# zeehu/generative_ranking_recommender

Measured on NVIDIA B200. Metric: RQ-KMeans vectors/sec per iteration (512-d, [128,128,256]), higher is better.
Workload: dtype 3xTF32 distance (fp32 accumulate), fp16 auction, fp32 centroids

## Files before the change

generative_ranking_recommender_b200/csrc/auction.cu:

```cuda
#include "common.cuh"

namespace rqk {

constexpr int AUC_W = 256;
constexpr int AUC_HALF = AUC_W / 2;
constexpr int AUC_NBUF = 3;
constexpr int AUC_BPL = AUC_W / 32;
constexpr int AUC_NW = 16;
constexpr int AUC_THREADS = AUC_NW * 32;
constexpr int AUC_BASE_CTAS = 296;
constexpr int AUC_MAX_CTAS = 1024;
constexpr int AUC_MAX_JOBS_PER_CTA = 65024;
constexpr int AUC_MIN_TILES_PER_CTA = 2;
constexpr int AUC_COLD_SHIFT = 8;
constexpr int AUC_MIN_KEY = 0x0400;
constexpr int AUC_SUB = 4096;
constexpr int AUC_QCAP = 256;
constexpr int AUC_SAMPLE_MAX = 8192;
constexpr int AUC_SEG_CAP = 256;
constexpr int AUC_KH = 128;
constexpr int AUC_SAMPLE_THREADS = 512;

enum { MODE_HIST = 0, MODE_BID = 1, MODE_DONE = 2 };

__device__ __forceinline__ void pdl_launch_dependents() { asm volatile("griddepcontrol.launch_dependents;" ::: "memory"); }
__device__ __forceinline__ void pdl_wait() { asm volatile("griddepcontrol.wait;" ::: "memory"); }

struct AuctionState {
    int mode;
    int counter;
    int rounds;
    int done;
    int ff_pending;
    int frozen_exit;
    int passes;
    int cold_passes;
    int window_misses;
    unsigned int eps_bits;
    unsigned int smax_bits, smin_bits;
    int need_sample;
    int error;
    int use_list;
    int force_scan;
    int list_passes;
    int sink[4];
    int branch[4];
    int pad_[4];
};

struct AuctionPtrs {
    AuctionState* st;
    __half* cost;
    short* owner;
    __half* sown;
    unsigned int* hist_g;
    unsigned int* above_g;
    unsigned int* gap_g;
    unsigned int* n_with;
    unsigned int* n_viol;
    unsigned int* tie_total;
    int* win_base;
    int* win_hbase;
    int* win_nlo;
    int* win_shift;
    int* tkey;
    int* take;
    int* tprev;
    int* miss_run;
    unsigned int* tieprefix;
    unsigned short* hist_cta;
    unsigned int* seg_list;
    unsigned int* seg_cnt;
    int* list_ok;
    unsigned int* rank_off;
    unsigned int* ticket;
    int* res_pass;
    unsigned int* above_cta;
    unsigned int* gap_cta;
    int* unres_g;
};

static inline int auction_tile_cols(int K) { return K <= 128 ? 128 : 64; }

static inline int auction_grid(long long N, int K) {
    long long tiles = ceil_div<long long>(N, auction_tile_cols(K));
    long long g = ceil_div<long long>(tiles, AUC_MIN_TILES_PER_CTA);
    const char* e = getenv("RQK_AUCTION_GRID");
    const int cap = (e && atoi(e) >= 1 && atoi(e) <= AUC_BASE_CTAS) ? atoi(e) : AUC_BASE_CTAS;
    if (g > cap) g = cap;
    long long g16 = ceil_div<long long>(N, AUC_MAX_JOBS_PER_CTA);
    if (g < g16) g = g16;
    if (g < 1) g = 1;
    return (int)g;
}

static inline int auction_spc(long long N, int K) {
    const int J = auction_tile_cols(K), G = auction_grid(N, K);
    const long long tiles = ceil_div<long long>(N, J);
    const long long len = ceil_div<long long>(tiles, G) * J;
    return (int)ceil_div<long long>(len, AUC_SUB);
}

static inline size_t auction_ws_layout(long long N, long long ld, int K, AuctionPtrs* p, char* base,
                                       size_t* reduce_off = nullptr, size_t* tie_total_off = nullptr) {
    int G = auction_grid(N, K);
    size_t off = 0;
    auto take_ = [&](size_t bytes) { size_t o = off; off += align256(bytes); return o; };
    size_t o_st = take_(sizeof(AuctionState));
    size_t o_cost = take_((size_t)ld * 2);
    size_t o_own = take_((size_t)ld * 2);
    size_t o_sown = take_((size_t)ld * 2);
    size_t o_hist = take_(((size_t)K * AUC_W + 2 * K + 2) * 4);
    size_t o_tt = take_((size_t)K * 4);
    size_t o_wb = take_((size_t)K * 4);
    size_t o_whb = take_((size_t)K * 4);
    size_t o_wnl = take_((size_t)K * 4);
    size_t o_ws = take_((size_t)K * 4);
    size_t o_tk = take_((size_t)K * 4);
    size_t o_take = take_((size_t)K * 4);
    size_t o_tprev = take_((size_t)K * 4);
    size_t o_mr = take_((size_t)K * 4);
    size_t o_tp = take_((size_t)G * K * 4);
    size_t o_hc = take_((size_t)G * K * AUC_W * 2);
    const size_t nseg = (size_t)G * auction_spc(N, K);
    size_t o_sl = take_(nseg * K * AUC_SEG_CAP * 4);
    size_t o_sc = take_(nseg * K * 4);
    size_t o_lo = take_(4);
    size_t o_ro = take_((size_t)K * 4);
    size_t o_tk2 = take_(4);
    size_t o_rp = take_((size_t)K * 4);
    size_t o_ac = take_((size_t)G * K * 4);
    size_t o_gc = take_((size_t)G * K * 4);
    size_t o_ug = take_(16);
    if (reduce_off) *reduce_off = o_hist;
    if (tie_total_off) *tie_total_off = o_tt;
    if (p) {
        p->st = (AuctionState*)(base + o_st);
        p->cost = (__half*)(base + o_cost);
        p->owner = (short*)(base + o_own);
        p->sown = (__half*)(base + o_sown);
        p->hist_g = (unsigned int*)(base + o_hist);
        p->above_g = p->hist_g + (size_t)K * AUC_W;
        p->gap_g = p->above_g + K;
        p->n_with = p->gap_g + K;
        p->n_viol = p->n_with + 1;
        p->tie_total = (unsigned int*)(base + o_tt);
        p->win_base = (int*)(base + o_wb);
        p->win_hbase = (int*)(base + o_whb);
        p->win_nlo = (int*)(base + o_wnl);
        p->win_shift = (int*)(base + o_ws);
        p->tkey = (int*)(base + o_tk);
        p->take = (int*)(base + o_take);
        p->tprev = (int*)(base + o_tprev);
        p->miss_run = (int*)(base + o_mr);
        p->tieprefix = (unsigned int*)(base + o_tp);
        p->hist_cta = (unsigned short*)(base + o_hc);
        p->seg_list = (unsigned int*)(base + o_sl);
        p->seg_cnt = (unsigned int*)(base + o_sc);
        p->list_ok = (int*)(base + o_lo);
        p->rank_off = (unsigned int*)(base + o_ro);
        p->ticket = (unsigned int*)(base + o_tk2);
        p->res_pass = (int*)(base + o_rp);
        p->above_cta = (unsigned int*)(base + o_ac);
        p->gap_cta = (unsigned int*)(base + o_gc);
        p->unres_g = (int*)(base + o_ug);
    }
    return off;
}

__global__ void auction_init_kernel(AuctionPtrs p, long long ld, int K, const unsigned int* minmax_keys, int force_scan) {
    long long i = (long long)blockIdx.x * blockDim.x + threadIdx.x;
    long long stride = (long long)gridDim.x * blockDim.x;
    for (long long j = i; j < ld; j += stride) {
        p.cost[j] = __ushort_as_half(0);
        p.owner[j] = -1;
    }
    for (long long j = i; j < (long long)K * AUC_W + 2 * K + 2; j += stride) p.hist_g[j] = 0;
    for (long long j = i; j < K; j += stride) {
        p.win_base[j] = 0;
        p.win_hbase[j] = AUC_HALF;
        p.win_nlo[j] = AUC_HALF;
        p.win_shift[j] = AUC_COLD_SHIFT;
        p.tkey[j] = -1;
        p.take[j] = 0;
        p.tprev[j] = -1;
        p.miss_run[j] = 0;
        p.rank_off[j] = 0;
        p.res_pass[j] = -1;
    }
    if (i == 0) {
        AuctionState s;
        memset(&s, 0, sizeof(s));
        s.mode = MODE_HIST;
        s.need_sample = 1;
        s.force_scan = force_scan;
        *p.list_ok = 1;
        *p.ticket = 0;
        p.unres_g[0] = 0;
        p.unres_g[1] = 0;
        p.unres_g[2] = 0;
// ... 851 lines not shown
                uint4 bufA[4], bufB[4];
                int a = warp, st = 0;
                int w = a < nact ? (int)acth[a] : 0;
                if (a < nact) load_step(w, 0, bufA);
                auto body = [&](uint4 (&cur)[4], uint4 (&nxt)[4]) {
                    int an = a, wn = w, sn = st + 1;
                    if (sn == nsteps) { an = a + AUC_NW; sn = 0; wn = an < nact ? (int)acth[an] : 0; }
                    if (an < nact) load_step(wn, sn, nxt);
                    const __half2 f2 = u2h2(sm.r_lo2[w]);
                    const uint4* cp = reinterpret_cast<const uint4*>(cost_s) + (st << 7) + lane;
                    unsigned int acc = 0;
#pragma unroll
                    for (int q = 0; q < 4; ++q) {
                        const uint4 cv = cp[q * 32];
                        const unsigned int sw[4] = {cur[q].x, cur[q].y, cur[q].z, cur[q].w};
                        const unsigned int cw[4] = {cv.x, cv.y, cv.z, cv.w};
#pragma unroll
                        for (int h = 0; h < 4; ++h) {
                            const __half2 v2 = __hsub2(u2h2(sw[h]), u2h2(cw[h]));
                            acc |= __hge2_mask(v2, f2) & ((1u << (4 * q + h)) | (1u << (16 + 4 * q + h)));
                        }
                    }
                    const int mine = __popc(acc);
                    int incl = mine;
#pragma unroll
                    for (int d = 1; d < 32; d <<= 1) {
                        const int o = __shfl_up_sync(0xffffffffu, incl, d);
                        if (lane >= d) incl += o;
                    }
                    const int total = __shfl_sync(0xffffffffu, incl, 31);
                    if (total) {
                        const int cbase = (st << 10) + lane * 8;
                        if (qn + total > AUC_QCAP) flush(w);
                        if (total <= AUC_QCAP) {
                            int pos = qn + incl - mine;
                            while (acc) {
                                const int bpos = __ffs(acc) - 1;
                                acc &= acc - 1;
                                const int pq = bpos & 15;
                                wq[pos++] = (unsigned short)(cbase + ((pq >> 2) << 8) + ((pq & 3) << 1) + (bpos >> 4));
                            }
                            qn += total;
                        } else {
                            while (__any_sync(0xffffffffu, acc != 0)) {
                                const int pc = __popc(acc);
                                const int take = pc < 4 ? pc : 4;
                                int in2 = take;
#pragma unroll
                                for (int d = 1; d < 32; d <<= 1) {
                                    const int o = __shfl_up_sync(0xffffffffu, in2, d);
                                    if (lane >= d) in2 += o;
                                }
                                int pos = in2 - take;
                                for (int r = 0; r < take; ++r) {
                                    const int bpos = __ffs(acc) - 1;
                                    acc &= acc - 1;
                                    const int pq = bpos & 15;
                                    wq[pos++] = (unsigned short)(cbase + ((pq >> 2) << 8) + ((pq & 3) << 1) + (bpos >> 4));
                                }
                                qn = __shfl_sync(0xffffffffu, in2, 31);
                                flush(w);
                            }
                        }
                    }
                    if (sn == 0 && qn) flush(w);
                    a = an;
                    w = wn;
                    st = sn;
                };
                while (a < nact) {
                    body(bufA, bufB);
#pragma unroll
                    for (int q = 0; q < 4; ++q) bufA[q] = bufB[q];
                }
            } else {
                for (int a = warp; a < nact; a += AUC_NW) {
                    const int w = acth[a];
                    const __half* srow = S + (size_t)w * ld + sub;
                    const int wbase = sm.r_base[w];
                    if (wbase > 0) {
                        const int whb = sm.r_hbase[w], wnlo = sm.r_nlo[w], wshift = sm.r_shift[w];
                        const __half lo = bits2h(key2h((unsigned)wbase));
                        for (int c0 = 0; c0 < sublen; c0 += 32) {
                            const int cc = c0 + lane;
                            bool live = cc < sublen;
                            if (live) live = __hge(__hsub(srow[cc], __ushort_as_half(cost_s[cc])), lo);
                            if (__any_sync(0xffffffffu, live)) emit(w, srow, live, live ? cc : 0, wbase, whb, wnlo, wshift);
                        }
                    } else {
                        const int shift = sm.r_shift[w];
                        for (int c0 = 0; c0 < sublen; c0 += 32) {
                            const int cc = c0 + lane;
                            const bool valid = cc < sublen;
                            __half v = __ushort_as_half(0xfc00);
                            if (valid) {
                                const __half sx = srow[cc];
                                v = (own_s[cc] == w) ? sx : __hsub(sx, __ushort_as_half(cost_s[cc]));
                            }
                            const int bin = (int)h2key(h2bits(v)) >> shift;
                            const bool hb = valid && bin < AUC_W;
                            const bool ab = valid && bin >= AUC_W;
                            unsigned int na = __popc(__ballot_sync(0xffffffffu, ab));
                            if (lane == 0 && na) atomicAdd(&sm.above[w], na);
                            unsigned int actm = __ballot_sync(0xffffffffu, hb);
                            if (actm) {
                                int lead = __ffs(actm) - 1;
                                int lbin = __shfl_sync(0xffffffffu, bin, lead);
                                unsigned int same = __ballot_sync(0xffffffffu, hb && bin == lbin);
                                if (same == actm) {
                                    if (lane == lead) hist_add(sm.hist, w - h0, lbin, __popc(actm));
                                } else if (hb) {
                                    hist_add(sm.hist, w - h0, bin);
                                }
                            }
                        }
                    }
                }
            }
            __syncthreads();
            if (tid >= h0 && tid < h0 + AUC_KH && tid < K && sm.r_shift[tid] != 0xff) {
                const unsigned int c = seg_cnt_s[tid];
                p.seg_cnt[(size_t)seg * K + tid] = c;
                if (c > AUC_SEG_CAP) *p.list_ok = 0;
            }
        }

        unsigned int* dump = reinterpret_cast<unsigned int*>(p.hist_cta + ((size_t)b * K + h0) * AUC_W);
        for (int a = tid >> 7; a < nact; a += AUC_THREADS >> 7) {
            const int i = ((int)acth[a] - h0) * (AUC_W / 2) + (tid & 127);
            const unsigned int h = sm.hist[i];
            dump[i] = h;
            if (!fused) {
                const int ig = h0 * (AUC_W / 2) + i;
                if (h & 0xffffu) atomicAdd(&p.hist_g[2 * ig], h & 0xffffu);
                if (h >> 16) atomicAdd(&p.hist_g[2 * ig + 1], h >> 16);
            }
        }
        ffh = 0;
    }

    const int nact_all = s_act_off[2];
    for (int a = tid; a < nact_all; a += AUC_THREADS) {
        const int i = act[a];
        if (fused) {
            p.above_cta[(size_t)b * K + i] = sm.above[i];
            p.gap_cta[(size_t)b * K + i] = sm.gap[i];
        } else {
            if (sm.above[i]) atomicAdd(&p.above_g[i], sm.above[i]);
            if (sm.gap[i]) atomicAdd(&p.gap_g[i], sm.gap[i]);
        }
    }
}

__global__ void __launch_bounds__(AUC_THREADS, 2)
auction_bidlist_kernel(const __half* __restrict__ S, long long ld, long long N, int K, int J, int spc, AuctionPtrs p,
                       long long n_global, int fused) {
    pdl_launch_dependents();
    pdl_wait();
    const AuctionState st = *p.st;
    if (st.mode != MODE_BID || !st.use_list) return;
    constexpr int NCH = AUC_SEG_CAP / 32;
    __shared__ __align__(16) unsigned int colmax[AUC_SUB];
    __shared__ __align__(16) short own_s[AUC_SUB];
    __shared__ __align__(16) unsigned char colviol[AUC_SUB];
    __shared__ unsigned int tie_seen[256];
    __shared__ int r_take[256], r_tk[256];
    __shared__ unsigned int s_nwith, s_nviol;
    const int tid = threadIdx.x, lane = tid & 31, warp = tid >> 5;
    const int counter = st.counter;
    const __half eps = bits2h(st.eps_bits);
    const unsigned int eps_bits = st.eps_bits;
    const bool retain = counter >= 1 && counter < 100;
    const bool fallback = counter > 1000;
    const int G = gridDim.x, b = blockIdx.x;
    const long long tiles_total = (N + J - 1) / J;
    const long long c_begin = (tiles_total * b / G) * J;
    long long c_end = (tiles_total * (b + 1) / G) * J;
    if (c_end > N) c_end = N;

    for (int i = tid; i < K; i += AUC_THREADS) {
        tie_seen[i] = p.tieprefix[(size_t)b * K + i];
        r_tk[i] = p.tkey[i];
        r_take[i] = p.take[i];
    }
    if (tid == 0) { s_nwith = 0; s_nviol = 0; }

    int seg = b * spc;
    for (long long sub = c_begin; sub < c_end; sub += AUC_SUB, ++seg) {
        const int sublen = (int)((c_end - sub) < AUC_SUB ? (c_end - sub) : AUC_SUB);
        static_assert(AUC_SUB == 8 * AUC_THREADS, "one 8-job group per thread");
        const int j0 = tid * 8;
        const bool grp = j0 < sublen;
        uint4 c8 = make_uint4(0u, 0u, 0u, 0u), o8 = make_uint4(0xffffffffu, 0xffffffffu, 0xffffffffu, 0xffffffffu);
        if (grp) {
            c8 = *reinterpret_cast<const uint4*>(p.cost + sub + j0);
            o8 = *reinterpret_cast<const uint4*>(p.owner + sub + j0);
        }
        {
            const unsigned int ow[4] = {o8.x, o8.y, o8.z, o8.w};
            unsigned int init[8];
#pragma unroll
            for (int e = 0; e < 8; ++e) {
                const int o = (int)(short)((ow[e >> 1] >> ((e & 1) * 16)) & 0xffffu);
                unsigned int v = 0;
                if (j0 + e < sublen) {
                    if (o >= 0) { if (retain) v = (eps_bits << 16) | (0xffffu - (unsigned)o); }
                    else if (fallback) v = (eps_bits << 16) | 0xffffu;
                }
                init[e] = v;
            }
            *reinterpret_cast<uint4*>(own_s + j0) = o8;
            *reinterpret_cast<uint4*>(colmax + j0) = make_uint4(init[0], init[1], init[2], init[3]);
            *reinterpret_cast<uint4*>(colmax + j0 + 4) = make_uint4(init[4], init[5], init[6], init[7]);
            *reinterpret_cast<uint2*>(colviol + j0) = make_uint2(0u, 0u);
        }
        __syncthreads();
        const int nrows = (K - warp + AUC_NW - 1) / AUC_NW;
        unsigned int E_l = (lane < nrows) ? __ldcg(p.seg_cnt + (size_t)seg * K + warp + AUC_NW * lane) : 0u;
        if (E_l > AUC_SEG_CAP) E_l = AUC_SEG_CAP;
        unsigned int pre0 = 0, pre1 = 0;
        {
            const unsigned int E0 = __shfl_sync(0xffffffffu, E_l, 0);
            const unsigned int* L0 = p.seg_list + ((size_t)seg * K + warp) * AUC_SEG_CAP;
            if ((unsigned)lane < E0) pre0 = __ldcg(L0 + lane);
            if ((unsigned)lane + 32 < E0) pre1 = __ldcg(L0 + 32 + lane);
        }
        for (int r = 0; r < nrows; ++r) {
            const int w = warp + AUC_NW * r;
            const unsigned int E = __shfl_sync(0xffffffffu, E_l, r);
            const unsigned int* L = p.seg_list + ((size_t)seg * K + w) * AUC_SEG_CAP;
            const int tk = r_tk[w];
            const __half T = bits2h(key2h((unsigned)tk));
            unsigned int ent[NCH], tmask[NCH];
            unsigned int n_ties = 0;
            ent[0] = pre0;
            ent[1] = pre1;
#pragma unroll
            for (int c = 2; c < NCH; ++c) {
                ent[c] = 0u;
                if ((unsigned)(c * 32) < E) {
                    const unsigned int idx = c * 32 + lane;
                    if (idx < E) ent[c] = __ldcg(L + idx);
                }
            }
            pre0 = 0; pre1 = 0;
            if (r + 1 < nrows) {
                const unsigned int En = __shfl_sync(0xffffffffu, E_l, r + 1);
                const unsigned int* Ln = L + (size_t)AUC_NW * AUC_SEG_CAP;
                if ((unsigned)lane < En) pre0 = __ldcg(Ln + lane);
                if ((unsigned)lane + 32 < En) pre1 = __ldcg(Ln + 32 + lane);
            }
#pragma unroll
            for (int c = 0; c < NCH; ++c) {
                tmask[c] = 0u;
                if ((unsigned)(c * 32) < E) {
                    const unsigned int idx = c * 32 + lane;
                    tmask[c] = __ballot_sync(0xffffffffu, idx < E && (int)(ent[c] & 0xffffu) == tk);
                    n_ties += __popc(tmask[c]);
                }
            }
            const unsigned int seen0 = tie_seen[w];
            const long long quota = r_take[w];
            const bool all_rej = (long long)seen0 >= quota;
            const bool all_acc = (long long)seen0 + n_ties <= quota;
            unsigned int rank[NCH];
#pragma unroll
            for (int c = 0; c < NCH; ++c) rank[c] = 0;
            if (n_ties && !all_rej && !all_acc) {
#pragma unroll
                for (int c = 0; c < NCH; ++c) {
                    unsigned int m = tmask[c];
                    while (m) {
                        const int src = __ffs(m) - 1;
                        m &= m - 1;
                        const unsigned int jsrc = __shfl_sync(0xffffffffu, ent[c], src) >> 16;
#pragma unroll
                        for (int c2 = 0; c2 < NCH; ++c2) rank[c2] += ((ent[c2] >> 16) > jsrc) ? 1u : 0u;
                    }
                }
            }
#pragma unroll
            for (int c = 0; c < NCH; ++c) {
                if ((unsigned)(c * 32) >= E) break;
                const unsigned int idx = c * 32 + lane;
                if (idx >= E) continue;
                const int key = (int)(ent[c] & 0xffffu);
                const int cc = (int)(ent[c] >> 16);
                bool bidder = key > tk;
                if (key == tk) bidder = all_acc || (!all_rej && (long long)seen0 + rank[c] < quota);
                if (!bidder) continue;
                const int o = own_s[cc];
                const bool own = (o == w);
                if (fallback && w == 0 && o < 0) continue;
                const __half v = bits2h(key2h((unsigned)key));
                unsigned int bid = h2bits(__hadd(__hsub(v, T), eps));
                if (retain && own) bid = eps_bits;
                if (!own) colviol[cc] = 1;
                atomicMax(&colmax[cc], (bid << 16) | (0xffffu - (unsigned)w));
            }
            if (lane == 0) tie_seen[w] = seen0 + n_ties;
        }
        __syncthreads();
        {
            const uint4 pa = *reinterpret_cast<const uint4*>(colmax + j0), pb = *reinterpret_cast<const uint4*>(colmax + j0 + 4);
            const uint2 vi = *reinterpret_cast<const uint2*>(colviol + j0);
            const unsigned int pk[8] = {pa.x, pa.y, pa.z, pa.w, pb.x, pb.y, pb.z, pb.w};
            const unsigned int cw[4] = {c8.x, c8.y, c8.z, c8.w}, ow[4] = {o8.x, o8.y, o8.z, o8.w};
            unsigned short sv[8];
            unsigned int changed = 0;
#pragma unroll
            for (int e = 0; e < 8; ++e) {
                sv[e] = 0;
                const int old_owner = (int)(short)((ow[e >> 1] >> ((e & 1) * 16)) & 0xffffu);
                if (pk[e]) {
                    const int wnr = (int)(0xffffu - (pk[e] & 0xffffu));
                    if (wnr != old_owner) {
                        changed |= 1u << e;
                        sv[e] = __half_as_ushort(S[(size_t)wnr * ld + sub + j0 + e]);
                    }
                }
            }
            unsigned int nc[4], no[4];
            int n_has = 0, n_vv = 0;
            bool cost_dirty = false, own_dirty = false;
#pragma unroll
            for (int e = 0; e < 8; ++e) {
                const int sh = (e & 1) * 16;
                unsigned int c = (cw[e >> 1] >> sh) & 0xffffu, o = (ow[e >> 1] >> sh) & 0xffffu;
                const int old_owner = (int)(short)o;
                bool vv = ((e < 4 ? vi.x >> (8 * e) : vi.y >> (8 * (e - 4))) & 0xffu) != 0;
                if (pk[e]) {
                    ++n_has;
                    c = h2bits(__hadd(__ushort_as_half((unsigned short)c), bits2h(pk[e] >> 16)));
                    cost_dirty = true;
                    if ((changed >> e) & 1u) { o = 0xffffu - (pk[e] & 0xffffu); own_dirty = true; }
                } else if (old_owner >= 0) {
                    o = 0xffffu;
                    own_dirty = true;
                    vv = true;
                }
                n_vv += vv ? 1 : 0;
                if (e & 1) { nc[e >> 1] |= c << 16; no[e >> 1] |= o << 16; }
                else { nc[e >> 1] = c; no[e >> 1] = o; }
            }
            if (grp) {
                if (cost_dirty) *reinterpret_cast<uint4*>(p.cost + sub + j0) = make_uint4(nc[0], nc[1], nc[2], nc[3]);
                if (own_dirty) *reinterpret_cast<uint4*>(p.owner + sub + j0) = make_uint4(no[0], no[1], no[2], no[3]);
#pragma unroll
                for (int e = 0; e < 8; ++e)
                    if ((changed >> e) & 1u) p.sown[sub + j0 + e] = __ushort_as_half(sv[e]);
            }
            n_has = __reduce_add_sync(0xffffffffu, n_has);
            n_vv = __reduce_add_sync(0xffffffffu, n_vv);
            if (lane == 0) {
                if (n_has) atomicAdd(&s_nwith, (unsigned)n_has);
                if (n_vv) atomicAdd(&s_nviol, (unsigned)n_vv);
            }
        }
        __syncthreads();
    }
    if (tid == 0) {
        if (s_nwith) atomicAdd(p.n_with, s_nwith);
        if (s_nviol) atomicAdd(p.n_viol, s_nviol);
    }
    if (fused && auction_last_cta(p.ticket)) auction_resolve_body(p, n_global, K, n_global / K, MODE_BID);
}

static inline size_t auction_pass_smem(int K, int J) {
    return (size_t)AUC_NBUF * K * J * 2 + (size_t)K * 16 + (size_t)J * 4 +
           (size_t)J * 4 + (size_t)K * 2 + (size_t)J + 64;
}

constexpr int AUC_SAMPLE = AUC_SAMPLE_MAX;
__device__ __forceinline__ void sample_select_bin(const unsigned int* hist, int base, int need, int* out_bin, int* out_above) {
    const int lane = threadIdx.x & 31;
    int h[8], lsum = 0;
#pragma unroll
    for (int i = 0; i < 8; ++i) { h[i] = (int)hist[lane * 8 + i]; lsum += h[i]; }
    int suf = lsum;
#pragma unroll
    for (int d = 1; d < 32; d <<= 1) {
        const int o = __shfl_down_sync(0xffffffffu, suf, d);
        if (lane + d < 32) suf += o;
    }
    int c = base + suf - lsum, bin = -1, above = 0;
#pragma unroll
    for (int i = 7; i >= 0; --i) {
        if (bin < 0 && c + h[i] >= need) { bin = lane * 8 + i; above = c; }
        c += h[i];
    }
    const unsigned int who = __ballot_sync(0xffffffffu, bin >= 0);
    int rb = 0, ra = base + __shfl_sync(0xffffffffu, suf, 0);
    if (who) {
        const int src = 31 - __clz(who);
        rb = __shfl_sync(0xffffffffu, bin, src);
        ra = __shfl_sync(0xffffffffu, above, src);
    }
    if (lane == 0) { *out_bin = rb; *out_above = ra; }
    *out_bin = rb;
    *out_above = ra;
}



__global__ void __launch_bounds__(AUC_SAMPLE_THREADS, 2)
auction_sample_kernel(const __half* __restrict__ S, long long ld, long long N, int K, long long jpw, AuctionPtrs p,
                      unsigned short* __restrict__ collect_out, int collect_n,
                      const unsigned short* __restrict__ ext_keys, int ext_n, int ext_cnt, PeerCtx peers, int peer_seq) {
    pdl_launch_dependents();
    pdl_wait();
    const AuctionState st = *p.st;
    if (st.mode != MODE_HIST || !st.need_sample) return;
    __shared__ unsigned short keys[AUC_SAMPLE];
    const int w = blockIdx.x, tid = threadIdx.x;
    if (peers.world > 0) {
        if (!peer_barrier(peers, 0, peer_seq, blockIdx.x == 0)) {
            if (tid == 0) { p.st->error = 1; p.st->mode = MODE_DONE; p.st->done = 1; }
            return;
        }
    }
    long long ns = N < AUC_SAMPLE ? N : AUC_SAMPLE;
    if (collect_out) ns = collect_n < ns ? collect_n : ns;
    if (ext_keys || peers.world > 0) ns = ext_n;
    const __half eps = bits2h(st.eps_bits);
    {
        constexpr int PER = 8;
        static_assert(AUC_SAMPLE % (PER * AUC_SAMPLE_THREADS) == 0, "whole batches");
        const long long nchunks = (ns + 15) / 16, cstride = N / (nchunks > 0 ? nchunks : 1);
        for (int q0 = 0; q0 < AUC_SAMPLE / AUC_SAMPLE_THREADS; q0 += PER) {
            __half c_r[PER], s_r[PER];
            short o_r[PER];
            unsigned short k_r[PER];
#pragma unroll
            for (int q = 0; q < PER; ++q) {
                const int i = tid + (q0 + q) * AUC_SAMPLE_THREADS;
                k_r[q] = 0;
                c_r[q] = s_r[q] = __ushort_as_half(0);
                o_r[q] = -1;
                if (ext_keys || peers.world > 0) {
                    if (i < ns) {
                        if (peers.world > 0)
                            k_r[q] = __ldcv(peer_sample(peers, i / ext_cnt, K, peer_seq & 1) + (size_t)w * ext_cnt + (i % ext_cnt));
                        else
                            k_r[q] = ext_keys[((size_t)(i / ext_cnt) * K + w) * ext_cnt + (i % ext_cnt)];
                    }
                } else if (i < ns) {
                    long long col = cstride * (i >> 4) + (i & 15);
                    if (col >= N) col = N - 1;
                    c_r[q] = p.cost[col];
                    o_r[q] = p.owner[col];
                    s_r[q] = S[(size_t)w * ld + col];
                }
            }
#pragma unroll
// ... 476 lines not shown
    if (s_mode != MODE_HIST) return;
    if (p.tkey[w] < 0) {
        unsigned int abt, gpt;
        merge_worker_dumps(p, K, G, w, m, &abt, &gpt);
        unsigned int* mine = peer_hist(peers, peers.rank, K, seq & 1);
        if (tid < AUC_W) mine[(size_t)w * AUC_W + tid] = m.hist[tid];
        if (tid == 0) { mine[(size_t)K * AUC_W + w] = abt; mine[(size_t)K * AUC_W + K + w] = gpt; }
    }
    __threadfence_system();
    __syncthreads();
    if (tid == 0) {
        const int t = atomicAdd(&p.unres_g[2], 1);
        s_mode = (t == (int)gridDim.x - 1) ? 1 : 0;
        if (s_mode) p.unres_g[2] = 0;
    }
    __syncthreads();
    if (s_mode && tid < peers.world && tid != peers.rank) {
        __threadfence_system();
        int* dst = peer_flags(peers, tid) + 1 * PEER_MAX + peers.rank;
        asm volatile("st.release.sys.global.s32 [%0], %1;" ::"l"(dst), "r"(seq) : "memory");
    }
}

__global__ void __launch_bounds__(AUC_MAX_CTAS, 1)
auction_peer_resolve_workers_kernel(AuctionPtrs p, int K, int G, long long jpw, PeerCtx peers, int seq) {
    pdl_launch_dependents();
    pdl_wait();
    __shared__ MergeSmem m;
    __shared__ unsigned int s_rows[PEER_MAX][AUC_W];
    __shared__ unsigned int s_abgp[2][PEER_MAX];
    __shared__ int s_flag[2], s_mode, s_passes;
    const int w = blockIdx.x, tid = threadIdx.x, warp = tid >> 5, par = seq & 1;
    if (tid == 0) { s_mode = p.st->mode; s_passes = p.st->passes; s_flag[0] = 0; s_flag[1] = 0; }
    __syncthreads();
    if (s_mode != MODE_HIST) return;
    const bool settled = p.tkey[w] >= 0;
    if (!settled) {
        if (!peer_barrier(peers, 1, seq, false)) {
            if (tid == 0) { p.st->error = 1; p.st->mode = MODE_DONE; p.st->done = 1; }
            return;
        }
        for (int i = tid; i < PEER_MAX * AUC_W; i += AUC_MAX_CTAS) {
            const int r = i / AUC_W, b = i % AUC_W;
            unsigned int v = 0;
            if (r < peers.world) {
                const unsigned int* src = peer_hist(peers, r, K, par) + (size_t)w * AUC_W + b;
                v = (r == peers.rank) ? __ldcg(src) : __ldcv(src);
            }
            s_rows[r][b] = v;
        }
        if (tid < 2 * PEER_MAX) {
            const int r = tid % PEER_MAX, which = tid / PEER_MAX;
            unsigned int v = 0;
            if (r < peers.world) {
                const unsigned int* src = peer_hist(peers, r, K, par) + (size_t)K * AUC_W + (size_t)which * K + w;
                v = (r == peers.rank) ? __ldcg(src) : __ldcv(src);
            }
            s_abgp[which][r] = v;
        }
        __syncthreads();
        if (tid < AUC_W) {
            unsigned int t = 0;
#pragma unroll
            for (int r = 0; r < PEER_MAX; ++r) t += s_rows[r][tid];
            m.hist[tid] = t;
        }
        __syncthreads();
        if (warp == 0) {
            unsigned long long abt = 0, gpt = 0;
#pragma unroll
            for (int r = 0; r < PEER_MAX; ++r) { abt += s_abgp[0][r]; gpt += s_abgp[1][r]; }
            resolve_worker_from_smem(p, w, m, abt, gpt, jpw, s_passes, s_flag);
        }
        __syncthreads();
        const int tk = p.tkey[w];
        if (tk >= 0) {
            const int base = p.win_base[w], hbase = p.win_hbase[w], nlo = p.win_nlo[w];
            const int bin = tk >= hbase ? nlo + tk - hbase : tk - base;
            unsigned int off = 0;
            for (int r = 0; r < peers.rank; ++r) off += s_rows[r][bin];
            if (tid == 0) p.rank_off[w] = off;
            tie_prefix_worker(p, K, G, w, m, off);
        }
        if (tid == 0) {
            if (s_flag[0]) atomicAdd(&p.unres_g[0], 1);
            if (s_flag[1]) atomicAdd(&p.unres_g[1], 1);
        }
    }
    if (auction_last_cta(p.ticket) && tid == 0) merge_state_transition(p);
}

__global__ void auction_tie_offset_kernel(AuctionPtrs p, int K, int G, const int* __restrict__ totals, int rank) {
    if (p.st->mode != MODE_BID) return;
    int i = blockIdx.x * blockDim.x + threadIdx.x;
    if (i < G * K) {
        unsigned int off = 0;
        for (int r = 0; r < rank; ++r) off += (unsigned int)totals[r * K + i % K];
        p.tieprefix[i] += off;
    }
}

__global__ void auction_finalize_kernel(AuctionPtrs p, long long N, int* __restrict__ assign) {
    long long i = (long long)blockIdx.x * blockDim.x + threadIdx.x;
    if (i < N) {
        short o = p.owner[i];
        assign[i] = o >= 0 ? (int)o : 0;
    }
}

}

namespace rqk {
struct AuctionArgs {
    AuctionPtrs p;
    int G, J;
    size_t smem;
};
static int auction_prepare(int64_t n, int64_t ld, int32_t k, void* workspace, size_t workspace_bytes, AuctionArgs* a,
                           const char* who) {
    if (!workspace) return fail(RQK_ERR_ARG, "%s: null workspace", who);
    if (k < 1 || k > 256) return fail(RQK_ERR_UNSUPPORTED, "%s: k=%lld outside [1,256]", who, k);
    if (n < 1) return fail(RQK_ERR_ARG, "%s: n=%lld < 1", who, n);
    if (ld % 128 != 0 || ld < n) return fail(RQK_ERR_ARG, "%s: ld=%lld must be a multiple of 128 and >= n", who, ld);
    size_t need = auction_ws_layout(n, ld, k, &a->p, (char*)workspace);
    if (workspace_bytes < need) return fail(RQK_ERR_WORKSPACE, "%s: workspace %lld < %lld bytes", who, (long long)workspace_bytes, (long long)need);
    a->G = auction_grid(n, k);
    if (a->G > AUC_MAX_CTAS) return fail(RQK_ERR_UNSUPPORTED, "%s: n=%lld jobs per GPU exceed the 66 M limit of this build", who, n);
    a->J = auction_tile_cols(k);
    a->smem = auction_pass_smem(k, a->J);
    return 0;
}

template <typename... KArgs, typename... Args>
static cudaError_t launch_round_kernel(void (*kernel)(KArgs...), unsigned grid, unsigned block, size_t smem,
                                       cudaStream_t stream, bool pdl, Args... args) {
    cudaLaunchConfig_t cfg = {};
    cfg.gridDim = dim3(grid);
    cfg.blockDim = dim3(block);
    cfg.dynamicSmemBytes = smem;
    cfg.stream = stream;
    cudaLaunchAttribute attr[1];
    attr[0].id = cudaLaunchAttributeProgrammaticStreamSerialization;
    attr[0].val.programmaticStreamSerializationAllowed = 1;
    cfg.attrs = attr;
    cfg.numAttrs = pdl ? 1 : 0;
    return cudaLaunchKernelEx(&cfg, kernel, KArgs(args)...);
}

static bool auction_list_refine_ok() {
    static const bool ok = [] { const char* e = getenv("RQK_AUCTION_NO_LIST_REFINE"); return !(e && e[0] == '1'); }();
    return ok;
}

static bool auction_pdl_ok() {
    static const bool ok = [] { const char* e = getenv("RQK_NO_PDL"); return !(e && e[0] == '1'); }();
    return ok;
}

static int auction_launch(const AuctionArgs& a, const void* scores_t, int64_t ld, int64_t n, int32_t k, int64_t n_global,
                          int which, int fused, cudaStream_t stream, bool chain = false) {
    const bool pdl = (fused != 0 || chain) && auction_pdl_ok();
    auto kern = (a.J == 128) ? auction_pass_kernel<128> : auction_pass_kernel<64>;
    int devi = 0;
    RQK_CUDA_OK(cudaGetDevice(&devi));
    devi &= RQK_MAX_DEVICES - 1;
    static size_t smem_set[RQK_MAX_DEVICES][2] = {};
    size_t& cur = smem_set[devi][a.J == 128 ? 0 : 1];
    if (a.smem > cur) {
        RQK_CUDA_OK(cudaFuncSetAttribute(kern, cudaFuncAttributeMaxDynamicSharedMemorySize, (int)a.smem));
        cur = a.smem;
    }
    const int spc = auction_spc(n, k);
    if (which & 1)
        RQK_CUDA_OK(launch_round_kernel(auction_sample_kernel, (unsigned)k, (unsigned)AUC_SAMPLE_THREADS, 0, stream, pdl, (const __half*)scores_t,
                                        (long long)ld, (long long)n, (int)k, (long long)(n_global / k), a.p,
                                        (unsigned short*)nullptr, 0, (const unsigned short*)nullptr, 0, 1, PeerCtx{}, 0));
    if (which & 2) {
        static bool hs_set[RQK_MAX_DEVICES] = {};
        const size_t hs = HistSmem::TOTAL;
        if (!hs_set[devi]) {
            RQK_CUDA_OK(cudaFuncSetAttribute(auction_hist_kernel, cudaFuncAttributeMaxDynamicSharedMemorySize, (int)hs));
            hs_set[devi] = true;
        }
        RQK_CUDA_OK(launch_round_kernel(auction_hist_kernel, (unsigned)a.G, (unsigned)AUC_THREADS, hs, stream, pdl,
                                        (const __half*)scores_t, (long long)ld, (long long)n, (int)k, a.J, spc, a.p,
                                        (long long)n_global, fused));
    }
    if (which & 8)
        RQK_CUDA_OK(launch_round_kernel(auction_merge_resolve_kernel, (unsigned)k, (unsigned)AUC_MAX_CTAS, 0, stream, pdl,
                                        a.p, (int)k, a.G, (long long)(n_global / k), spc, auction_list_refine_ok() ? 1 : 0));
    if (which & 4) {
        RQK_CUDA_OK(launch_round_kernel(auction_bidlist_kernel, (unsigned)a.G, (unsigned)AUC_THREADS, 0, stream, pdl,
                                        (const __half*)scores_t, (long long)ld, (long long)n, (int)k, a.J, spc, a.p,
                                        (long long)n_global, fused));
        RQK_CUDA_OK(launch_round_kernel(kern, (unsigned)a.G, (unsigned)AUC_THREADS, a.smem, stream, pdl,
                                        (const __half*)scores_t, (long long)ld, (long long)n, (int)k, (long long)(n_global / k),
                                        a.p, (long long)n_global, fused));
    }
    RQK_LAUNCH_OK();
    return 0;
}
}

extern "C" {

struct rqk_auction_layout {
    int64_t total_bytes;
    int64_t reduce_offset;
    int64_t reduce_count;
    int64_t tie_total_offset;
};

struct rqk_auction_info {
    int32_t done;
    int32_t rounds;
    int32_t passes;
    int32_t cold_passes;
    int32_t window_misses;
    int32_t frozen_exit;
    int32_t counter;
    uint16_t eps_bits;
    uint16_t list_passes;
};

int rqk_auction_layout_query(int64_t n, int32_t k, rqk_auction_layout* out) {
    using namespace rqk;
    if (!out || n < 1 || k < 1 || k > 256) return fail(RQK_ERR_ARG, "rqk_auction_layout_query: bad argument%s");
    long long ld = round_up<long long>(n, 128);
    size_t ro = 0, to = 0;
    out->total_bytes = (int64_t)auction_ws_layout(n, ld, k, nullptr, nullptr, &ro, &to);
    out->reduce_offset = (int64_t)ro;
    out->reduce_count = (int64_t)k * AUC_W + 2 * k + 2;
    out->tie_total_offset = (int64_t)to;
    return 0;
}

size_t rqk_auction_workspace_bytes(int64_t n, int32_t k) {
    long long ld = rqk::round_up<long long>(n, 128);
    return rqk::auction_ws_layout(n, ld, k, nullptr, nullptr);
}

int rqk_auction_init(int64_t n, int64_t ld, int32_t k, const void* minmax_keys, void* workspace,
                     size_t workspace_bytes, void* stream_) {
    using namespace rqk;
    AuctionArgs a;
    int rc = auction_prepare(n, ld, k, workspace, workspace_bytes, &a, "rqk_auction_init");
    if (rc) return rc;
    if (!minmax_keys) return fail(RQK_ERR_ARG, "rqk_auction_init: null minmax_keys%s");
    cudaStream_t stream = (cudaStream_t)stream_;
    RQK_CUDA_OK(cudaMemsetAsync(a.p.tieprefix, 0, (size_t)a.G * k * 4, stream));
    const char* ns = getenv("RQK_AUCTION_NO_LIST");
    auction_init_kernel<<<148, 256, 0, stream>>>(a.p, ld, k, (const unsigned int*)minmax_keys, (ns && ns[0] == '1') ? 1 : 0);
    RQK_LAUNCH_OK();
    return 0;
}

int rqk_auction_pass(const void* scores_t, int64_t ld, int64_t n, int32_t k, int64_t n_global, int32_t which,
                     void* workspace, size_t workspace_bytes, void* stream_) {
    using namespace rqk;
    AuctionArgs a;
    int rc = auction_prepare(n, ld, k, workspace, workspace_bytes, &a, "rqk_auction_pass");
    if (rc) return rc;
    if (!scores_t) return fail(RQK_ERR_ARG, "rqk_auction_pass: null scores%s");
    if (n_global < k) return fail(RQK_ERR_ARG, "rqk_auction_pass: n_global=%s%lld < k=%lld (argmin path, reference :24-26)", "", n_global, k);
    if (which == 0) which = 7;
    if (n_global != n) which &= ~1;
    const int fused = (which & 16) && n_global == n ? 1 : 0;
    if ((which & 8) && !fused) return fail(RQK_ERR_ARG, "rqk_auction_pass: bit 3 (merge + resolve) needs bit 4 and unsharded jobs%s");
    return auction_launch(a, scores_t, ld, n, k, n_global, which & 15, fused, (cudaStream_t)stream_);
}

int rqk_auction_sample_collect(const void* scores_t, int64_t ld, int64_t n, int32_t k, int64_t n_global, void* out,
                               int32_t count, void* workspace, size_t workspace_bytes, void* stream_) {
    using namespace rqk;
    AuctionArgs a;
    int rc = auction_prepare(n, ld, k, workspace, workspace_bytes, &a, "rqk_auction_sample_collect");
    if (rc) return rc;
    if (!scores_t || !out || count < 1 || count > AUC_SAMPLE) return fail(RQK_ERR_ARG, "rqk_auction_sample_collect: bad argument%s");
    auction_sample_kernel<<<k, AUC_SAMPLE_THREADS, 0, (cudaStream_t)stream_>>>((const __half*)scores_t, ld, n, k, n_global / k, a.p,
                                                                  (unsigned short*)out, count, nullptr, 0, 1, PeerCtx{}, 0);
    RQK_LAUNCH_OK();
    return 0;
}

int rqk_auction_sample_window(int64_t n, int64_t ld, int32_t k, int64_t n_global, const void* keys, int32_t count,
                              int32_t parts, void* workspace, size_t workspace_bytes, void* stream_) {
    using namespace rqk;
    AuctionArgs a;
    int rc = auction_prepare(n, ld, k, workspace, workspace_bytes, &a, "rqk_auction_sample_window");
    if (rc) return rc;
    if (!keys || count < 1 || parts < 1 || (int64_t)count * parts > AUC_SAMPLE)
        return fail(RQK_ERR_ARG, "rqk_auction_sample_window: bad argument%s");
    auction_sample_kernel<<<k, AUC_SAMPLE_THREADS, 0, (cudaStream_t)stream_>>>(nullptr, ld, n_global, k, n_global / k, a.p, nullptr, 0,
                                                                  (const unsigned short*)keys, count * parts, count, PeerCtx{}, 0);
    RQK_LAUNCH_OK();
    return 0;
}

int rqk_auction_resolve(int64_t n, int64_t ld, int32_t k, int64_t n_global, int32_t expect, void* workspace,
                        size_t workspace_bytes, void* stream_) {
    using namespace rqk;
    AuctionArgs a;
    int rc = auction_prepare(n, ld, k, workspace, workspace_bytes, &a, "rqk_auction_resolve");
    if (rc) return rc;
    cudaStream_t stream = (cudaStream_t)stream_;
    if (expect < -1 || expect > 1) return fail(RQK_ERR_ARG, "rqk_auction_resolve: expect must be -1, 0 or 1%s");
    auction_resolve_kernel<<<1, 1024, 0, stream>>>(a.p, n_global, k, n_global / k, expect);
    auction_tieprefix_kernel<<<k, AUC_MAX_CTAS, 0, stream>>>(a.p, k, a.G);
    RQK_LAUNCH_OK();
    return 0;
}

size_t rqk_auction_peer_bytes(int32_t k) { return rqk::peer_bytes(k); }

static int peer_ctx(const void* const* peers, int32_t world, int32_t rank, rqk::PeerCtx* c, const char* who) {
    using namespace rqk;
    if (!peers || world < 1 || world > PEER_MAX || rank < 0 || rank >= world)
        return fail(RQK_ERR_ARG, "%s: bad peer arguments (world 1..8)", who);
    for (int r = 0; r < PEER_MAX; ++r) c->buf[r] = r < world ? (unsigned char*)peers[r] : nullptr;
    for (int r = 0; r < world; ++r)
        if (!c->buf[r]) return fail(RQK_ERR_ARG, "%s: null peer pointer", who);
    c->world = world;
    c->rank = rank;
    return 0;
}

int rqk_auction_peer_round(const void* scores_t, int64_t ld, int64_t n, int32_t k, int64_t n_global, int32_t count,
                           const void* const* peers, int32_t world, int32_t rank, int32_t seq0, void* workspace,
                           size_t workspace_bytes, void* stream_) {
    using namespace rqk;
    AuctionArgs a;
    int rc = auction_prepare(n, ld, k, workspace, workspace_bytes, &a, "rqk_auction_peer_round");
    if (rc) return rc;
    PeerCtx c;
    if ((rc = peer_ctx(peers, world, rank, &c, "rqk_auction_peer_round"))) return rc;
    if (!scores_t || count < 1 || (int64_t)count * world > AUC_SAMPLE) return fail(RQK_ERR_ARG, "rqk_auction_peer_round: bad argument%s");
    if (n_global < k) return fail(RQK_ERR_ARG, "rqk_auction_peer_round: n_global=%s%lld < k=%lld", "", n_global, k);
    cudaStream_t stream = (cudaStream_t)stream_;
    const bool pdl = auction_pdl_ok();
    RQK_CUDA_OK(launch_round_kernel(auction_peer_bid_collect_kernel, (unsigned)k, 1024u, 0, stream, pdl, (const __half*)scores_t,
                                    (long long)ld, (long long)n, (int)k, (long long)n_global, a.p, (int)count, c, (int)seq0,
                                    (int)(seq0 + 1)));
    RQK_CUDA_OK(launch_round_kernel(auction_sample_kernel, (unsigned)k, (unsigned)AUC_SAMPLE_THREADS, 0, stream, pdl, (const __half*)nullptr, (long long)ld,
                                    (long long)n_global, (int)k, (long long)(n_global / k), a.p, (unsigned short*)nullptr, 0,
                                    (const unsigned short*)nullptr, (int)(count * world), (int)count, c, (int)(seq0 + 1)));
    if ((rc = auction_launch(a, scores_t, ld, n, k, n_global, 2, 1, stream, true))) return rc;
    RQK_CUDA_OK(launch_round_kernel(auction_peer_publish_kernel, (unsigned)k, (unsigned)AUC_MAX_CTAS, 0, stream, pdl, a.p, (int)k,
// ... 118 lines not shown
```

Baseline: 196.4 million.

## Stage bid-list segments in shared memory via cp.async with batched processing

Restructures the auction bid-list kernel so that, instead of each warp walking rows with per-lane global loads and warp ballots, all per-worker segment lists are copied into dynamically sized shared memory with cp.async in prefix-sum-packed batches. Tie counting and bidding are then done flat over 16-byte chunks by all threads. It also hoists loads that do not depend on the prior kernel ahead of the PDL state check. In exchange it adds a large dynamic shared allocation (about 78KB), which may limit occupancy. Tie ranking becomes an O(cnt) scan per tied entry, and a global atomic counter is added for batch statistics.

New measurement: 201.7 million, median of 6. +2.7%, better.

```diff
diff --git a/generative_ranking_recommender_b200/csrc/auction.cu b/generative_ranking_recommender_b200/csrc/auction.cu
--- a/generative_ranking_recommender_b200/csrc/auction.cu
+++ b/generative_ranking_recommender_b200/csrc/auction.cu
@@ -45,7 +45,8 @@
     int list_passes;
     int sink[4];
     int branch[4];
-    int pad_[4];
+    int list_batches;
+    int pad_[3];
 };
 
 struct AuctionPtrs {
@@ -1203,50 +1204,78 @@
     }
 }
 
+constexpr int AUC_STAGE_CHUNKS = 4608;
+static_assert(AUC_STAGE_CHUNKS >= AUC_SEG_CAP / 4, "a batch holds at least one whole segment");
+static_assert(AUC_SEG_CAP * 4 % 16 == 0, "segments start 16-byte aligned");
+__host__ __device__ constexpr size_t auction_stage_smem(int chunks) { return (size_t)chunks * 17; }
+
 __global__ void __launch_bounds__(AUC_THREADS, 2)
 auction_bidlist_kernel(const __half* __restrict__ S, long long ld, long long N, int K, int J, int spc, AuctionPtrs p,
-                       long long n_global, int fused) {
+                       long long n_global, int fused, int stage_chunks) {
     pdl_launch_dependents();
     pdl_wait();
+    const int tid = threadIdx.x, lane = tid & 31, warp = tid >> 5;
+    const int G = gridDim.x, b = blockIdx.x;
+    const long long tiles_total = (N + J - 1) / J;
+    const long long c_begin = (tiles_total * b / G) * J;
+    long long c_end = (tiles_total * (b + 1) / G) * J;
+    if (c_end > N) c_end = N;
+    static_assert(AUC_SUB == 8 * AUC_THREADS, "one 8-job group per thread");
+    static_assert(AUC_THREADS >= 256, "one thread per worker");
+    const int j0 = tid * 8;
+    uint4 c8, o8;
+    unsigned int E;
+    auto load_sub = [&](long long sub, int seg) {
+        c8 = make_uint4(0u, 0u, 0u, 0u);
+        o8 = make_uint4(0xffffffffu, 0xffffffffu, 0xffffffffu, 0xffffffffu);
+        if (sub + j0 < c_end) {
+            c8 = *reinterpret_cast<const uint4*>(p.cost + sub + j0);
+            o8 = *reinterpret_cast<const uint4*>(p.owner + sub + j0);
+        }
+        E = (tid < K) ? __ldcg(p.seg_cnt + (size_t)seg * K + tid) : 0u;
+    };
+    load_sub(c_begin, b * spc);
+    unsigned int w_seen = 0;
+    int w_tk = 0, w_take = 0;
+    if (tid < K) {
+        w_seen = p.tieprefix[(size_t)b * K + tid];
+        w_tk = p.tkey[tid];
+        w_take = p.take[tid];
+    }
     const AuctionState st = *p.st;
     if (st.mode != MODE_BID || !st.use_list) return;
-    constexpr int NCH = AUC_SEG_CAP / 32;
+    extern __shared__ __align__(16) unsigned char bl_dyn[];
+    uint4* stage = reinterpret_cast<uint4*>(bl_dyn);
+    unsigned char* stage_w = bl_dyn + (size_t)stage_chunks * 16;
     __shared__ __align__(16) unsigned int colmax[AUC_SUB];
     __shared__ __align__(16) short own_s[AUC_SUB];
     __shared__ __align__(16) unsigned char colviol[AUC_SUB];
     __shared__ unsigned int tie_seen[256];
     __shared__ int r_take[256], r_tk[256];
+    __shared__ int s_cnt[256];
+    __shared__ int s_off[257];
+    __shared__ int s_ties[256];
+    __shared__ int s_wsum[AUC_NW];
     __shared__ unsigned int s_nwith, s_nviol;
-    const int tid = threadIdx.x, lane = tid & 31, warp = tid >> 5;
     const int counter = st.counter;
     const __half eps = bits2h(st.eps_bits);
     const unsigned int eps_bits = st.eps_bits;
     const bool retain = counter >= 1 && counter < 100;
     const bool fallback = counter > 1000;
-    const int G = gridDim.x, b = blockIdx.x;
-    const long long tiles_total = (N + J - 1) / J;
-    const long long c_begin = (tiles_total * b / G) * J;
-    long long c_end = (tiles_total * (b + 1) / G) * J;
-    if (c_end > N) c_end = N;
-
-    for (int i = tid; i < K; i += AUC_THREADS) {
-        tie_seen[i] = p.tieprefix[(size_t)b * K + i];
-        r_tk[i] = p.tkey[i];
-        r_take[i] = p.take[i];
-    }
-    if (tid == 0) { s_nwith = 0; s_nviol = 0; }
+
+    if (tid < K) {
+        tie_seen[tid] = w_seen;
+        r_tk[tid] = w_tk;
+        r_take[tid] = w_take;
+    }
+    if (tid == 0) { s_nwith = 0; s_nviol = 0; s_off[0] = 0; }
 
     int seg = b * spc;
     for (long long sub = c_begin; sub < c_end; sub += AUC_SUB, ++seg) {
         const int sublen = (int)((c_end - sub) < AUC_SUB ? (c_end - sub) : AUC_SUB);
-        static_assert(AUC_SUB == 8 * AUC_THREADS, "one 8-job group per thread");
-        const int j0 = tid * 8;
         const bool grp = j0 < sublen;
-        uint4 c8 = make_uint4(0u, 0u, 0u, 0u), o8 = make_uint4(0xffffffffu, 0xffffffffu, 0xffffffffu, 0xffffffffu);
-        if (grp) {
-            c8 = *reinterpret_cast<const uint4*>(p.cost + sub + j0);
-            o8 = *reinterpret_cast<const uint4*>(p.owner + sub + j0);
-        }
+        if (sub != c_begin) load_sub(sub, seg);
+        if (E > AUC_SEG_CAP) E = AUC_SEG_CAP;
         {
             const unsigned int ow[4] = {o8.x, o8.y, o8.z, o8.w};
             unsigned int init[8];
@@ -1265,92 +1294,95 @@
             *reinterpret_cast<uint4*>(colmax + j0 + 4) = make_uint4(init[4], init[5], init[6], init[7]);
             *reinterpret_cast<uint2*>(colviol + j0) = make_uint2(0u, 0u);
         }
+        unsigned int inc = (E + 3) >> 2;
+#pragma unroll
+        for (int d = 1; d < 32; d <<= 1) {
+            const unsigned int v = __shfl_up_sync(0xffffffffu, inc, d);
+            if (lane >= d) inc += v;
+        }
+        if (lane == 31) s_wsum[warp] = (int)inc;
         __syncthreads();
-        const int nrows = (K - warp + AUC_NW - 1) / AUC_NW;
-        unsigned int E_l = (lane < nrows) ? __ldcg(p.seg_cnt + (size_t)seg * K + warp + AUC_NW * lane) : 0u;
-        if (E_l > AUC_SEG_CAP) E_l = AUC_SEG_CAP;
-        unsigned int pre0 = 0, pre1 = 0;
-        {
-            const unsigned int E0 = __shfl_sync(0xffffffffu, E_l, 0);
-            const unsigned int* L0 = p.seg_list + ((size_t)seg * K + warp) * AUC_SEG_CAP;
-            if ((unsigned)lane < E0) pre0 = __ldcg(L0 + lane);
-            if ((unsigned)lane + 32 < E0) pre1 = __ldcg(L0 + 32 + lane);
-        }
-        for (int r = 0; r < nrows; ++r) {
-            const int w = warp + AUC_NW * r;
-            const unsigned int E = __shfl_sync(0xffffffffu, E_l, r);
-            const unsigned int* L = p.seg_list + ((size_t)seg * K + w) * AUC_SEG_CAP;
-            const int tk = r_tk[w];
-            const __half T = bits2h(key2h((unsigned)tk));
-            unsigned int ent[NCH], tmask[NCH];
-            unsigned int n_ties = 0;
-            ent[0] = pre0;
-            ent[1] = pre1;
-#pragma unroll
-            for (int c = 2; c < NCH; ++c) {
-                ent[c] = 0u;
-                if ((unsigned)(c * 32) < E) {
-                    const unsigned int idx = c * 32 + lane;
-                    if (idx < E) ent[c] = __ldcg(L + idx);
-                }
-            }
-            pre0 = 0; pre1 = 0;
-            if (r + 1 < nrows) {
-                const unsigned int En = __shfl_sync(0xffffffffu, E_l, r + 1);
-                const unsigned int* Ln = L + (size_t)AUC_NW * AUC_SEG_CAP;
-                if ((unsigned)lane < En) pre0 = __ldcg(Ln + lane);
-                if ((unsigned)lane + 32 < En) pre1 = __ldcg(Ln + 32 + lane);
-            }
-#pragma unroll
-            for (int c = 0; c < NCH; ++c) {
-                tmask[c] = 0u;
-                if ((unsigned)(c * 32) < E) {
-                    const unsigned int idx = c * 32 + lane;
-                    tmask[c] = __ballot_sync(0xffffffffu, idx < E && (int)(ent[c] & 0xffffu) == tk);
-                    n_ties += __popc(tmask[c]);
-                }
-            }
-            const unsigned int seen0 = tie_seen[w];
-            const long long quota = r_take[w];
-            const bool all_rej = (long long)seen0 >= quota;
-            const bool all_acc = (long long)seen0 + n_ties <= quota;
-            unsigned int rank[NCH];
-#pragma unroll
-            for (int c = 0; c < NCH; ++c) rank[c] = 0;
-            if (n_ties && !all_rej && !all_acc) {
-#pragma unroll
-                for (int c = 0; c < NCH; ++c) {
-                    unsigned int m = tmask[c];
-                    while (m) {
-                        const int src = __ffs(m) - 1;
-                        m &= m - 1;
-                        const unsigned int jsrc = __shfl_sync(0xffffffffu, ent[c], src) >> 16;
-#pragma unroll
-                        for (int c2 = 0; c2 < NCH; ++c2) rank[c2] += ((ent[c2] >> 16) > jsrc) ? 1u : 0u;
+        if (tid < K) {
+            for (int i = 0; i < warp; ++i) inc += s_wsum[i];
+            s_off[tid + 1] = (int)inc;
+            s_cnt[tid] = (int)E;
+        }
+        __syncthreads();
+        int nbatch = 0;
+        for (int wb = 0; wb < K; ++nbatch) {
+            const int base = s_off[wb];
+            const int we = wb + __syncthreads_count(tid >= wb && tid < K && s_off[tid + 1] - base <= stage_chunks);
+            for (int w = wb + warp; w < we; w += AUC_NW) {
+                const int c0 = s_off[w] - base, nc = s_off[w + 1] - s_off[w];
+                const unsigned int* L = p.seg_list + ((size_t)seg * K + w) * AUC_SEG_CAP;
+                for (int c = lane; c < nc; c += 32) {
+                    cp_async16(stage + c0 + c, L + 4 * c);
+                    stage_w[c0 + c] = (unsigned char)w;
+                }
+                if (lane == 0) s_ties[w] = 0;
+            }
+            cp_async_commit();
+            cp_async_wait<0>();
+            __syncthreads();
+            const int nch = s_off[we] - base;
+            for (int q = tid; q < nch; q += AUC_THREADS) {
+                const int w = stage_w[q];
+                const uint4 e4 = stage[q];
+                const int nv = s_cnt[w] - 4 * (q + base - s_off[w]);
+                const int tk = r_tk[w];
+                const int n = ((int)(e4.x & 0xffffu) == tk) + (nv > 1 && (int)(e4.y & 0xffffu) == tk) +
+                              (nv > 2 && (int)(e4.z & 0xffffu) == tk) + (nv > 3 && (int)(e4.w & 0xffffu) == tk);
+                if (n) atomicAdd(&s_ties[w], n);
+            }
+            __syncthreads();
+            for (int w = wb + tid; w < we; w += AUC_THREADS) {
+                const unsigned int seen0 = tie_seen[w];
+                const int n_ties = s_ties[w];
+                const long long rem = (long long)r_take[w] - seen0;
+                s_ties[w] = rem <= 0 ? 0 : (rem >= n_ties ? AUC_SEG_CAP : (int)rem);
+                tie_seen[w] = seen0 + n_ties;
+            }
+            __syncthreads();
+            for (int q = tid; q < nch; q += AUC_THREADS) {
+                const int w = stage_w[q];
+                const uint4 e4 = stage[q];
+                const int seg_c0 = s_off[w] - base;
+                const int cnt = s_cnt[w];
+                const int nv = cnt - 4 * (q - seg_c0);
+                const int tk = r_tk[w];
+                const int tie_bid = s_ties[w];
+                const __half T = bits2h(key2h((unsigned)tk));
+                const unsigned int ent[4] = {e4.x, e4.y, e4.z, e4.w};
+#pragma unroll
+                for (int i = 0; i < 4; ++i) {
+                    if (i >= nv) break;
+                    const int key = (int)(ent[i] & 0xffffu);
+                    const int cc = (int)(ent[i] >> 16);
+                    bool bidder = key > tk;
+                    if (key == tk) {
+                        bidder = tie_bid >= AUC_SEG_CAP;
+                        if (tie_bid > 0 && !bidder) {
+                            const unsigned int* se = reinterpret_cast<const unsigned int*>(stage + seg_c0);
+                            int rank = 0;
+                            for (int x = 0; x < cnt; ++x)
+                                rank += ((int)(se[x] & 0xffffu) == tk && (int)(se[x] >> 16) < cc) ? 1 : 0;
+                            bidder = rank < tie_bid;
+                        }
                     }
-                }
-            }
-#pragma unroll
-            for (int c = 0; c < NCH; ++c) {
-                if ((unsigned)(c * 32) >= E) break;
-                const unsigned int idx = c * 32 + lane;
-                if (idx >= E) continue;
-                const int key = (int)(ent[c] & 0xffffu);
-                const int cc = (int)(ent[c] >> 16);
-                bool bidder = key > tk;
-                if (key == tk) bidder = all_acc || (!all_rej && (long long)seen0 + rank[c] < quota);
-                if (!bidder) continue;
-                const int o = own_s[cc];
-                const bool own = (o == w);
-                if (fallback && w == 0 && o < 0) continue;
-                const __half v = bits2h(key2h((unsigned)key));
-                unsigned int bid = h2bits(__hadd(__hsub(v, T), eps));
-                if (retain && own) bid = eps_bits;
-                if (!own) colviol[cc] = 1;
-                atomicMax(&colmax[cc], (bid << 16) | (0xffffu - (unsigned)w));
-            }
-            if (lane == 0) tie_seen[w] = seen0 + n_ties;
-        }
+                    if (!bidder) continue;
+                    const int o = own_s[cc];
+                    const bool own = (o == w);
+                    if (fallback && w == 0 && o < 0) continue;
+                    const __half v = bits2h(key2h((unsigned)key));
+                    unsigned int bid = h2bits(__hadd(__hsub(v, T), eps));
+                    if (retain && own) bid = eps_bits;
+                    if (!own) colviol[cc] = 1;
+                    atomicMax(&colmax[cc], (bid << 16) | (0xffffu - (unsigned)w));
+                }
+            }
+            wb = we;
+        }
+        if (tid == 0 && nbatch > 1) atomicAdd(&p.st->list_batches, nbatch - 1);
         __syncthreads();
         {
             const uint4 pa = *reinterpret_cast<const uint4*>(colmax + j0), pb = *reinterpret_cast<const uint4*>(colmax + j0 + 4);
@@ -2133,6 +2165,12 @@
     return ok;
 }
 
+static int auction_stage_chunks() {
+    const char* e = getenv("RQK_AUCTION_LIST_STAGE");
+    const int c = e ? atoi(e) / 4 : 0;
+    return (c >= AUC_SEG_CAP / 4 && c < AUC_STAGE_CHUNKS) ? c : AUC_STAGE_CHUNKS;
+}
+
 static bool auction_pdl_ok() {
     static const bool ok = [] { const char* e = getenv("RQK_NO_PDL"); return !(e && e[0] == '1'); }();
     return ok;
@@ -2171,9 +2209,16 @@
         RQK_CUDA_OK(launch_round_kernel(auction_merge_resolve_kernel, (unsigned)k, (unsigned)AUC_MAX_CTAS, 0, stream, pdl,
                                         a.p, (int)k, a.G, (long long)(n_global / k), spc, auction_list_refine_ok() ? 1 : 0));
     if (which & 4) {
-        RQK_CUDA_OK(launch_round_kernel(auction_bidlist_kernel, (unsigned)a.G, (unsigned)AUC_THREADS, 0, stream, pdl,
-                                        (const __half*)scores_t, (long long)ld, (long long)n, (int)k, a.J, spc, a.p,
-                                        (long long)n_global, fused));
+        static bool bl_set[RQK_MAX_DEVICES] = {};
+        if (!bl_set[devi]) {
+            RQK_CUDA_OK(cudaFuncSetAttribute(auction_bidlist_kernel, cudaFuncAttributeMaxDynamicSharedMemorySize,
+                                             (int)auction_stage_smem(AUC_STAGE_CHUNKS)));
+            bl_set[devi] = true;
+        }
+        const int chunks = auction_stage_chunks();
+        RQK_CUDA_OK(launch_round_kernel(auction_bidlist_kernel, (unsigned)a.G, (unsigned)AUC_THREADS, auction_stage_smem(chunks),
+                                        stream, pdl, (const __half*)scores_t, (long long)ld, (long long)n, (int)k, a.J, spc,
+                                        a.p, (long long)n_global, fused, chunks));
         RQK_CUDA_OK(launch_round_kernel(kern, (unsigned)a.G, (unsigned)AUC_THREADS, a.smem, stream, pdl,
                                         (const __half*)scores_t, (long long)ld, (long long)n, (int)k, (long long)(n_global / k),
                                         a.p, (long long)n_global, fused));
```
